# DUNE/larnd-sim

Measured on AMD Instinct MI355X. Metric: edep segments/s end-to-end (quench->ADC), module0 config, higher is better.
Workload: dtype f64

## Files before the change

### larnd-sim_amd/csrc/chain.hip

```cpp
#include <stdio.h>
#include <math.h>

#include <vector>

#include "ldsim_args.h"
#include <utility>

int seg_launch_max_pixels(ldsim_ctx*, int64_t, int64_t, int32_t*, unsigned long long*);
int seg_launch_get_pixels(ldsim_ctx*, int64_t, int64_t, int, int32_t*, int, int32_t*, int32_t*, int, double*, const int32_t*,
                          int32_t);
int sort_make_keys(ldsim_ctx*, const int32_t*, const int32_t*, int64_t, int32_t, int, int64_t, unsigned long long*,
                   int32_t*, unsigned long long*);
int sort_pairs(ldsim_ctx*, unsigned long long*, unsigned long long*, int32_t*, int32_t*, int64_t);
int sort_pairs_bits(ldsim_ctx*, unsigned long long*, unsigned long long*, int32_t*, int32_t*, int64_t, int, int);
int sort_compact_valid(ldsim_ctx*, const unsigned long long*, int64_t, unsigned long long*, int32_t*, unsigned int*);
int sort_exclusive_scan_i32(ldsim_ctx*, const int32_t*, int32_t*, int64_t);
int sort_heads(ldsim_ctx*, const unsigned long long*, int64_t, int32_t*);
int sort_fill_unique(ldsim_ctx*, const unsigned long long*, const int32_t*, const int32_t*, int64_t, int32_t, int32_t*,
                     int32_t*, int64_t*, int64_t);
int sort_batch_first(ldsim_ctx*, int64_t, int64_t, int32_t, int32_t*);
int sort_tmax_batch(ldsim_ctx*, int64_t, int64_t, int32_t, double*, int32_t*, unsigned long long*);
int gform_launch(ldsim_ctx* ctx, const CurArgs& a, unsigned long long* counters, int32_t** flags_out,
                 const int32_t** flag_list, const unsigned long long** flag_count);
int sort_compact_hits(ldsim_ctx*, const int32_t*, const int32_t*, const int32_t*, const int32_t*, const double*,
// ... 307 lines not shown
  a.pixels = nullptr;
  a.seg_begin = seg_begin;
  a.P = P;
  a.n_pairs = n_valid;
  a.out = d_waves;
  a.T = T;
  a.tmax_batch = d_tmax_b;
  a.batch0 = batch0;
  a.batch_first = d_first_b;
  a.counters = counters;
  a.only_flagged = nullptr;
  a.flag_stride = 0;
  CK(ldsim_ensure(ctx, SB_WIN, (size_t)n_valid * 8 + 8));
  a.win = (int32_t*)ctx->scratch[SB_WIN].p;
  HIPCHK(hipEventRecord(ctx->ev[1], st));
  bool split_timed = false, win_used = false;
  CK(run_tracks_current(ctx, a, n, counters, &split_timed, &win_used));
  HIPCHK(hipEventRecord(ctx->ev[2], st));

  CK(ldsim_ensure(ctx, SB_ADC, (size_t)U * A * 8));
  CK(ldsim_ensure(ctx, SB_TICKS, (size_t)U * A * 8));
  CK(ldsim_ensure(ctx, SB_DIGIT, (size_t)U * A * 8));
  CK(ldsim_ensure(ctx, SB_TPM, (size_t)U * M * 8));
  CK(ldsim_ensure(ctx, SB_PAIRPIX, (size_t)U * 8 + 16));
  if (want_fractions) CK(ldsim_ensure(ctx, SB_FRAC, (size_t)U * A * M * 8));
  int32_t* d_hitcnt = (int32_t*)ctx->scratch[SB_PAIRPIX].p;
  int32_t* d_hitoff = d_hitcnt + U;
  FeeArgs F{};
  F.c = ctx->d_consts;
  F.k = FEEK_FROM(h);
  F.U = U;
  F.upix = d_upix; F.ubatch = d_ubatch; F.uoff = d_uoff;
  F.pair_val = d_vals2; F.pair_key = d_keys2;
  F.P = P;
  F.track_starts = d_starts;
  F.waves = d_waves;
  F.win = win_used ? (const int32_t*)ctx->scratch[SB_WIN].p : nullptr;
  F.T = T;
  F.batch_first = d_first_b;
  F.batch0 = batch0;
  F.threshold = h.discrimination_threshold * 1.0;
  F.thr_table = tables_fit ? ctx->d_pix_thr : nullptr;
  F.gain_table = tables_fit ? ctx->d_pix_gain : nullptr;
  F.time_padding = 0.0;
  F.adc_list = (double*)ctx->scratch[SB_ADC].p;
  F.adc_ticks = (double*)ctx->scratch[SB_TICKS].p;
  F.adc_digit = (double*)ctx->scratch[SB_DIGIT].p;
  F.tpm = (int64_t*)ctx->scratch[SB_TPM].p;
  F.fractions = want_fractions ? (double*)ctx->scratch[SB_FRAC].p : nullptr;
  F.counters = counters;
  F.hit_count = d_hitcnt;
  F.debug = ctx->debug_phases;
  const bool noisy = h.reset_noise_charge != 0 || h.uncorrelated_noise_charge != 0 || h.discriminator_noise != 0;
  const bool keyed_inline = noisy && ctx->rng_keyed && !ctx->debug_rng_materialize;
  if (keyed_inline) {
    F.batch_keys = (const uint64_t*)ctx->d_batch_keys.p;
    F.rng_seed = ctx->rng_seed;
  } else if (noisy && ctx->rng_keyed) {
    const int nd = rng_fee_draws_per_pixel(h, h.n_time_ticks);
    CK(ldsim_ensure(ctx, SB_NOISE, (size_t)U * nd * 4));
    CK(ldsim_ensure(ctx, SB_NDRAWS, (size_t)U * 4 + 4));
    CK(rng_launch_fee_keyed_fill(ctx, d_ubatch, d_upix, U, nd, (float*)ctx->scratch[SB_NOISE].p));
    F.noise_z = (const float*)ctx->scratch[SB_NOISE].p;
    F.noise_nd = nd;
    F.n_draws = (int32_t*)ctx->scratch[SB_NDRAWS].p;
  } else if (noisy) {
// ... 46 lines not shown
```

### larnd-sim_amd/csrc/kernels_fee.hip

```cpp
#include <algorithm>
#include "ldsim_args.h"
#include "rng.h"

#define FEE_THREADS 256
#define FEE_SPAN 512
#define NT_MAX 4096
#define A_MAX 64
#define M_MAX 64


template <int CTRL, int ROW_MASK>
__device__ __forceinline__ double dpp_or_zero(double v) {
  const int lo = __builtin_amdgcn_update_dpp(0, __double2loint(v), CTRL, ROW_MASK, 0xF, true);
  const int hi = __builtin_amdgcn_update_dpp(0, __double2hiint(v), CTRL, ROW_MASK, 0xF, true);
  return __hiloint2double(hi, lo);
}
__device__ __forceinline__ double wave_incl_scan(double v, int lane) {
  v += dpp_or_zero<0x111, 0xF>(v);
  v += dpp_or_zero<0x112, 0xF>(v);
  v += dpp_or_zero<0x114, 0xF>(v);
  v += dpp_or_zero<0x118, 0xF>(v);
  v += dpp_or_zero<0x142, 0xA>(v);
  v += dpp_or_zero<0x143, 0xC>(v);
  return v;
// ... 120 lines not shown
      adc = q_sum + (double)za * s_unc;
      disc2 = (double)zb * s_disc;
      cur += 2;
    }
    if (adc < thr + disc2) {
      ic += reset_ticks;
      q_sum = z ? (double)zs.get(cur++) * s_reset : 0.0;
      true_q = 0;
      last_reset = ic;
      adc_busy = 0;
      continue;
    }
    if (lane == 0) {
      int crossing = ic < n_time_ticks - 1 ? ic : n_time_ticks - 1;
      int post = ic - crossing > 0 ? ic - crossing : 0;
      double tt = (crossing == NT) ? t_stop : crossing * tstep;
      hits[iadc].lr = last_reset;
      hits[iadc].b = integrate_end;
      hits[iadc].q = adc;
      hits[iadc].tq = true_q;
      hits[iadc].tick = tt + time_padding - 2 + post;
    }
    ic += reset_ticks;
    last_reset = ic;
    adc_busy = busy_ticks;
    q_sum = z ? (double)zs.get(cur++) * s_reset : 0.0;
    true_q = 0;
    iadc++;
  }
  *n_draws = cur;
  return iadc;
}

template <int THREADS, bool KEYED = false>
__device__ __forceinline__ void pixel_adc_body(const FeeArgs& F, const int64_t u, const int32_t* __restrict__ span ,
                                               const int s_cap) {
  const FeeK* c = &F.k;
  const int tid = threadIdx.x, lane = tid & 63, wv = tid >> 6;
  const int NT = c->n_time_ticks;
  const int A = c->max_adc_values, M = c->max_tracks_per_pixel;
  const double dt = c->time_sampling, rt = c->buffer_risetime;

  extern __shared__ double S[];
  __shared__ HitRec hits[A_MAX];
  __shared__ int s_start[M_MAX], s_w0[M_MAX], s_w1[M_MAX];
  __shared__ int64_t s_row[M_MAX];
  __shared__ double wtap[64], G[64];
  __shared__ int s_nh, s_trange[2];

  const int64_t p0 = F.uoff[u], p1 = F.uoff[u + 1];
  __shared__ int s_nvalid;
  if (tid == 0) s_nvalid = 0;
  __syncthreads();
  {
    int cnt = 0;
    for (int64_t p = p0 + tid; p < p1; p += THREADS) cnt += (F.pair_key[p] & 15ull) != 15ull;
    if (cnt) atomicAdd(&s_nvalid, cnt);
  }
  __syncthreads();
  const int n_valid = s_nvalid;
  const int n_slots = n_valid < M ? n_valid : M;
  const bool overflow = (p1 - p0) > n_slots;
  const int ubatch = F.ubatch[u];
  const int bfirst = F.batch_first[ubatch - F.batch0];
  if (tid < n_slots) {
    int32_t v = F.pair_val[p0 + tid];
    int r = v / F.P;
    s_start[tid] = (int)py_round(F.track_starts[r] / dt);
    s_row[tid] = p0 + tid;
    s_w0[tid] = F.win ? F.win[2 * (p0 + tid)] : 0;
    s_w1[tid] = F.win ? F.win[2 * (p0 + tid) + 1] : F.T;
    F.tpm[u * M + tid] = r - bfirst;
  } else if (tid < M) {
    F.tpm[u * M + tid] = -1;
  }
  const int ntap = rt > 0 ? (int)ceil(10 * rt / dt) : 0;
  if (tid <= ntap && rt > 0) {
    wtap[tid] = exp((-tid) * dt / rt) * (1 - exp(-dt / rt));
  }
  __syncthreads();
  if (tid == 0) {
    double acc = 0;
    for (int d = 0; d <= ntap; d++) {
      acc += (rt > 0 ? wtap[d] : 1.0) * dt;
      G[d] = acc;
    }
  }
  const int s_lo = span ? span[2 * u] : 0;
  const int s_hi = span ? min(s_lo + s_cap, NT) : NT;
  for (int t = tid; t < s_hi - s_lo; t += THREADS) S[t] = 0;
  if (tid == 0) {
    int t_lo = NT, t_hi = 0;
    for (int k = 0; k < n_slots; k++) {
      const int lo = max(s_start[k] + s_w0[k], 0), hi = min(s_start[k] + s_w1[k], NT);
      if (hi > lo) { t_lo = min(t_lo, lo); t_hi = max(t_hi, hi); }
    }
    s_trange[0] = t_lo;
    s_trange[1] = t_hi;
  }
  for (int k = 0; k < n_slots && !(F.debug & 0x10000); k++) {
    const int st = s_start[k];
    const int lo = max(st + s_w0[k], 0), hi = min(st + s_w1[k], NT);
    const float* wf = F.waves + s_row[k] * (int64_t)F.T - st;
    for (int t = lo + ((tid - lo) & (THREADS - 1)); t < hi; t += THREADS) S[t - s_lo] += (double)wf[t];
  }
  __syncthreads();
  if (wv == 0) {
    const double thr = F.thr_table ? F.thr_table[F.upix[u]] : F.threshold;
    int nd = 0;
    int nh = 0;
    if (F.debug & 0x20000) {
    } else if (KEYED) {
      const KeyedNoise zs{F.rng_seed, key_mix(F.batch_keys[ubatch], (uint64_t)(int64_t)F.upix[u])};
      nh = adc_scan(c, S, NT, 1 * c->time_interval1, thr, F.time_padding, lane, hits, wtap, ntap, zs, &nd, s_trange[0],
                    s_trange[1], s_lo, s_hi);
    } else {
      const TableNoise zs{F.noise_z ? F.noise_z + u * (int64_t)F.noise_nd : nullptr};
      nh = adc_scan(c, S, NT, 1 * c->time_interval1, thr, F.time_padding, lane, hits, wtap, ntap, zs, &nd, s_trange[0],
                    s_trange[1], s_lo, s_hi);
    }
    if (lane == 0) {
      s_nh = nh;
      if (F.n_draws) F.n_draws[u] = nd;
    }
  }
  __syncthreads();
  const int nh = s_nh;
  const double gain = F.gain_table ? F.gain_table[F.upix[u]] : c->gain * (1e-3 * (1e-6 * 1.0)) / 1.0;
  for (int h = tid; h < A; h += THREADS) {
    double q = h < nh ? hits[h].q : 0.0;
    F.adc_list[u * A + h] = q;
    F.adc_ticks[u * A + h] = h < nh ? hits[h].tick : 0.0;
    F.adc_digit[u * A + h] = digitize_one(c, q, gain);
  }
  if (tid == 0) {
    F.hit_count[u] = nh;
    if (overflow) stat_add(F.counters, 2, 1ull);
    if (nh) stat_add(F.counters, 3, (unsigned long long)nh);
  }
  if (F.fractions && !(F.debug & 0x40000)) {
    double* fr = F.fractions + u * (int64_t)A * M;
    for (int k = wv; k < n_slots; k += THREADS / 64) {
      const float* wf = F.waves + s_row[k] * (int64_t)F.T;
      const int st = s_start[k];
      for (int h = 0; h < nh; h++) {
        int lr = hits[h].lr, b = hits[h].b;
        int hi = b < NT - 1 ? b : NT - 1;
        const int j0 = max(lr, st + s_w0[k]), j1 = min(hi, st + s_w1[k] - 1);
        double acc = 0;
        for (int jc = j0 + ((lr + lane - j0) & 63); jc <= j1; jc += 64) {
          int it = jc - st;
          int d = b - jc;
          acc += (double)wf[it] * (rt > 0 ? G[d < ntap ? d : ntap] : dt);
        }
        acc = wave_sum(acc);
        if (lane == 0) fr[h * M + k] = hits[h].tq > 0 ? acc / hits[h].tq : acc;
      }
    }
  }
}

template <int THREADS, bool KEYED = false>
__global__ void __launch_bounds__(THREADS) pixel_adc_kernel(FeeArgs F) {
  if ((int64_t)blockIdx.x < F.U) pixel_adc_body<THREADS, KEYED>(F, (int64_t)blockIdx.x, nullptr, 0);
}
template <int THREADS, bool KEYED = false>
__global__ void __launch_bounds__(THREADS) pixel_adc_list_kernel(FeeArgs F, const int32_t* __restrict__ list,
                                                                const unsigned long long* __restrict__ count,
                                                                const int32_t* __restrict__ span, int s_cap) {
  const int64_t n = (int64_t)*count;
  for (int64_t i = blockIdx.x; i < n; i += gridDim.x) {
    pixel_adc_body<THREADS, KEYED>(F, (int64_t)list[i], span, s_cap);
    __syncthreads();
  }
}

__global__ void __launch_bounds__(256) fee_clear_fractions_kernel(int64_t U, const int32_t* __restrict__ hit_count,
                                                                 const int64_t* __restrict__ tpm, int A, int M, double* __restrict__ fr) {
  const int64_t u = blockIdx.x;
  if (u >= U) return;
  __shared__ int s_ns;
  if (threadIdx.x == 0) s_ns = 0;
  __syncthreads();
  if ((int)threadIdx.x < M && tpm[u * M + threadIdx.x] != -1) atomicAdd(&s_ns, 1);
  __syncthreads();
  const int nh = hit_count[u], ns = s_ns;
  double* row = fr + u * (int64_t)A * M;
  for (int h = 0; h < A; h++)
    for (int k = threadIdx.x; k < M; k += 256)
      if (!(h < nh && k < ns)) row[h * M + k] = 0.0;
}

extern "C++" int fee_clear_unwritten_fractions(ldsim_ctx* ctx, int64_t U, const int32_t* hit_count, const int64_t* tpm, double* fr) {
  if (U == 0) return 0;
  const LdsimConsts& h = ctx->h_consts;
  hipLaunchKernelGGL(fee_clear_fractions_kernel, dim3((unsigned)U), dim3(256), 0, ctx->stream, U, hit_count, tpm,
                     h.max_adc_values, h.max_tracks_per_pixel, fr);
  HIPCHK(hipGetLastError());
  return 0;
}

__global__ void __launch_bounds__(256) fee_span_kernel(FeeArgs F, int32_t* __restrict__ span, int32_t* __restrict__ lists ,
                                                       unsigned long long* __restrict__ counts ) {
  const FeeK* c = &F.k;
  const int64_t u = (int64_t)blockIdx.x * 256 + threadIdx.x;
  const int lane = threadIdx.x & 63;
  int cls = -1;
  if (u < F.U) {
    const int NT = c->n_time_ticks, M = c->max_tracks_per_pixel;
    const double dt = c->time_sampling;
    const int64_t p0 = F.uoff[u], p1 = F.uoff[u + 1];
    int n_slots = 0;
    for (int64_t p = p0; p < p1 && n_slots < M; p++) n_slots += (F.pair_key[p] & 15ull) != 15ull;
    int t_lo = NT, t_hi = 0;
    for (int k = 0; k < n_slots; k++) {
      const int r = F.pair_val[p0 + k] / F.P;
      const int st = (int)py_round(F.track_starts[r] / dt);
      const int w0 = F.win ? F.win[2 * (p0 + k)] : 0, w1 = F.win ? F.win[2 * (p0 + k) + 1] : F.T;
      const int lo = max(st + w0, 0), hi = min(st + w1, NT);
      if (hi > lo) { t_lo = min(t_lo, lo); t_hi = max(t_hi, hi); }
    }
    if (t_hi <= t_lo) { t_lo = 0; t_hi = 0; }
    span[2 * u] = t_lo;
    span[2 * u + 1] = t_hi;
    cls = (t_hi - t_lo <= FEE_SPAN) ? 0 : 1;
  }
  for (int cc = 0; cc < 2; cc++) {
    const unsigned long long m = __ballot(cls == cc);
    if (!m) continue;
    unsigned long long base = 0;
    if (lane == 0) base = atomicAdd(&counts[cc], (unsigned long long)__popcll(m));
    base = ((unsigned long long)(unsigned)__builtin_amdgcn_readfirstlane((int)(base >> 32)) << 32) |
           (unsigned)__builtin_amdgcn_readfirstlane((int)base);
    if (cls == cc) lists[(int64_t)cc * F.U + (int64_t)base + __popcll(m & ((1ull << lane) - 1ull))] = (int32_t)u;
  }
}

extern "C++" int fee_launch_chain(ldsim_ctx* ctx, const FeeArgs& F) {
  if (F.U == 0) return 0;
  const LdsimConsts& h = ctx->h_consts;
  if (h.n_time_ticks > NT_MAX || h.max_adc_values > A_MAX || h.max_tracks_per_pixel > M_MAX ||
      (h.buffer_risetime > 0 && 10 * h.buffer_risetime / h.time_sampling > 62)) {
    ldsim_set_error("FEE constants exceed the kernel's static tiles");
    return LDSIM_EINVAL;
  }
  const size_t full = (size_t)((h.n_time_ticks + 1) & ~1) * 8;
  if (F.batch_keys) {
    hipLaunchKernelGGL((pixel_adc_kernel<FEE_THREADS, true>), dim3((unsigned)F.U), dim3(FEE_THREADS), full, ctx->stream, F);
    HIPCHK(hipGetLastError());
    return 0;
  }
  const bool skip_idle = !F.noise_z && ((F.thr_table != nullptr) || F.threshold > 0);
  if (!skip_idle || !F.win || ctx->fee_one_class || h.n_time_ticks <= FEE_SPAN) {
    hipLaunchKernelGGL(pixel_adc_kernel<FEE_THREADS>, dim3((unsigned)F.U), dim3(FEE_THREADS), full, ctx->stream, F);
    HIPCHK(hipGetLastError());
    return 0;
  }
  int rc;
  if ((rc = ldsim_ensure(ctx, SB_SPAN, (size_t)F.U * 16 + 64))) return rc;
  int32_t* d_span = (int32_t*)ctx->scratch[SB_SPAN].p;
  int32_t* d_lists = d_span + 2 * F.U;
  unsigned long long* d_counts = (unsigned long long*)((char*)ctx->scratch[SB_SPAN].p + (((size_t)F.U * 16 + 15) & ~(size_t)15));
  HIPCHK(hipMemsetAsync(d_counts, 0, 16, ctx->stream));
  hipLaunchKernelGGL(fee_span_kernel, dim3((unsigned)((F.U + 255) / 256)), dim3(256), 0, ctx->stream, F, d_span, d_lists, d_counts);
  HIPCHK(hipGetLastError());
  const unsigned g_small = (unsigned)std::min<int64_t>(F.U, 256 * 24), g_big = (unsigned)std::min<int64_t>(F.U, 256 * 8);
  hipLaunchKernelGGL(pixel_adc_list_kernel<64>, dim3(g_small), dim3(64), (size_t)FEE_SPAN * 8, ctx->stream, F, d_lists,
                     d_counts, d_span, FEE_SPAN);
  HIPCHK(hipGetLastError());
  hipLaunchKernelGGL(pixel_adc_list_kernel<FEE_THREADS>, dim3(g_big), dim3(FEE_THREADS), full, ctx->stream, F,
                     d_lists + F.U, d_counts + 1, (const int32_t*)nullptr, 0);
  HIPCHK(hipGetLastError());
  return 0;
}

__global__ void track_pixel_map_kernel(int64_t* map, const int32_t* unique_pix, int64_t U, const int32_t* pixels,
                                       const int32_t* dist, int64_t S, int P, int max_distance, int M) {
  int64_t u = (int64_t)blockIdx.x * blockDim.x + threadIdx.x;
  if (u >= U) return;
  int32_t upix = unique_pix[u];
  int64_t* row = map + u * M;
  for (int target = 0; target < max_distance; target++)
    for (int64_t itrk = 0; itrk < S; itrk++)
      for (int ipix = 0; ipix < P; ipix++) {
        if (upix != pixels[itrk * P + ipix]) continue;
        if (dist[itrk * P + ipix] == target) {
          int imap = 0;
          while (imap < M) {
            if (row[imap] == itrk) { imap = -1; break; }
            if (row[imap] == -1) break;
            imap++;
          }
          if (imap >= 0 && imap < M) row[imap] = itrk;
        }
        break;
      }
}

__global__ void sum_pixel_signals_kernel(double* pixels_signals, const float* signals, const double* track_starts,
                                         const int64_t* pim, const int64_t* tpm, double* pts, double* overflow,
                                         int64_t S, int P, int T, int NT, int M, double dt) {
  int64_t pairi = blockIdx.x;
  int64_t itrk = pairi / P;
  int64_t pidx = pim[pairi];
// ... 127 lines not shown
```

### larnd-sim_amd/csrc/ldsim_abi.hip

```cpp
#include <stdarg.h>
#include <stdio.h>
#include <string.h>

#include <algorithm>
#include <cmath>
#include <new>
#include <vector>

#include "ldsim_args.h"

struct CurArgs;
struct FeeArgs;
int seg_launch_unpack(ldsim_ctx*, const LdsimTrackLayout*, int64_t);
int seg_launch_repack(ldsim_ctx*, const LdsimTrackLayout*, int64_t);
int seg_launch_quench_drift(ldsim_ctx*, int, int, int, int*);
int seg_launch_quench_drift_map(ldsim_ctx*, int, int*);
int seg_launch_max_pixels(ldsim_ctx*, int64_t, int64_t, int32_t*, unsigned long long*);
int seg_launch_get_pixels(ldsim_ctx*, int64_t, int64_t, int, int32_t*, int, int32_t*, int32_t*, int, double*, const int32_t*,
                          int32_t);
int seg_launch_time_intervals(ldsim_ctx*, int64_t, int64_t, double*, int32_t*);
int fee_launch_track_pixel_map(ldsim_ctx*, int64_t*, const int32_t*, int64_t, const int32_t*, const int32_t*, int64_t,
                               int, int, int);
int fee_launch_sum_pixel_signals(ldsim_ctx*, double*, const float*, const double*, const int64_t*, const int64_t*,
                                 double*, double*, int64_t, int, int, int, int);
// ... 168 lines not shown
    (void)ldsim_ctx_destroy(ctx);
    return rc;
  }
  *out = ctx;
  return 0;
}

extern "C" int ldsim_set_consts(ldsim_ctx* ctx, const LdsimConsts* consts) {
  LDSIM_ENTER(ctx);
  NEED(ctx && consts, "null argument");
  CK(light_join(ctx));
  NEED(consts->n_tpc >= 0 && consts->n_tpc <= LDSIM_MAX_TPC, "n_tpc out of range");
  if (memcmp(&ctx->h_consts, consts, sizeof(LdsimConsts)) != 0) ctx->wbuf_learned = 0;
  ctx->h_consts = *consts;
  HIPCHK(hipMemcpyAsync(ctx->d_consts, &ctx->h_consts, sizeof(LdsimConsts), hipMemcpyHostToDevice, ctx->stream));
  HIPCHK(hipStreamSynchronize(ctx->stream));
  return 0;
}

extern "C" int ldsim_ctx_destroy(ldsim_ctx* ctx) {
  if (!ctx) return 0;
  {
    const std::thread::id me = std::this_thread::get_id();
    std::thread::id none{};
    if (ctx->owner.load(std::memory_order_acquire) != me && !ctx->owner.compare_exchange_strong(none, me, std::memory_order_acq_rel)) {
      ldsim_set_error("ctx in use by another thread: not destroyed");
      return LDSIM_ESTATE;
    }
  }
  (void)hipSetDevice(ctx->device);
  if (ctx->stream) (void)hipStreamSynchronize(ctx->stream);
  void* ptrs[] = {ctx->d_consts, ctx->d_resp,      ctx->d_eff,    ctx->d_ch2tpc, ctx->d_lut_vis, ctx->d_lut_t0,
                  ctx->d_lut_t0avg, ctx->d_lut_td, ctx->seg_block.p, ctx->raw.p,  ctx->d_pix_thr, ctx->d_pix_gain,
                  ctx->d_glx, ctx->d_glw, ctx->light_flag_dev};
  for (void* p : ptrs)
    if (p) (void)hipFree(p);
  if (ctx->copy_stream) {
    (void)hipStreamSynchronize(ctx->copy_stream);
    (void)hipStreamDestroy(ctx->copy_stream);
  }
  if (ctx->light_stream) {
    (void)hipStreamSynchronize(ctx->light_stream);
    (void)hipStreamDestroy(ctx->light_stream);
  }
  if (ctx->tab_stream) {
    (void)hipStreamSynchronize(ctx->tab_stream);
    (void)hipStreamDestroy(ctx->tab_stream);
  }
  for (auto& e : ctx->tab_ev)
    if (e) (void)hipEventDestroy(e);
  if (ctx->ev_light_in) (void)hipEventDestroy(ctx->ev_light_in);
  if (ctx->ev_light_done) (void)hipEventDestroy(ctx->ev_light_done);
  for (auto& b : ctx->scratch)
    if (b.p) (void)hipFree(b.p);
  for (auto& b : ctx->out_alt)
    if (b.p) (void)hipFree(b.p);
  for (int i = 0; i < 8; i++)
    if (ctx->ev[i]) (void)hipEventDestroy(ctx->ev[i]);
  for (int i = 0; i < 4; i++)
    if (ctx->evl[i]) (void)hipEventDestroy(ctx->evl[i]);
  for (DevBuf* b : {&ctx->light_nph, &ctx->light_t0, &ctx->light_vox, &ctx->light_out, &ctx->light_tid, &ctx->light_tph,
                    &ctx->light_opc, &ctx->light_trk, &ctx->light_scint, &ctx->light_scint_tid, &ctx->light_scint_tph,
                    &ctx->light_disc, &ctx->light_resp, &ctx->light_resp_tid, &ctx->light_resp_tph, &ctx->light_w[0],
                    &ctx->light_w[1], &ctx->light_gain, &ctx->resp_pad, &ctx->light_tmax, &ctx->light_env, &ctx->light_xd, &ctx->light_wtid, &ctx->light_wtph, &ctx->light_wtid2})
    if (b->p) (void)hipFree(b->p);
  for (auto& b : ctx->light_tmp)
    if (b.p) (void)hipFree(b.p);
// ... 1385 lines not shown
```

### larnd-sim_amd/csrc/ldsim_args.h

```cpp
#pragma once
#include "ldsim_dev.h"

#define STAT_STRIPES 64
#define STAT_WORDS (16 * (1 + STAT_STRIPES))
#define STAT_BYTES (8 * STAT_WORDS)
#define MISC_BYTES (256 + STAT_BYTES + 256)
#ifdef __HIPCC__
__device__ __forceinline__ void stat_add(unsigned long long* counters, int i, unsigned long long v) {
  atomicAdd(&counters[16 * (1 + (blockIdx.x & (STAT_STRIPES - 1))) + i], v);
}
#endif
static inline void stat_sum(const unsigned long long* raw, unsigned long long* sum16) {
  for (int i = 0; i < 16; i++) {
    sum16[i] = raw[i];
    for (int s = 0; s < STAT_STRIPES; s++) sum16[i] += raw[16 * (1 + s) + i];
  }
}

struct CurArgs {
  SegStore s;
  const LdsimConsts* c;
  const double* resp;
  int32_t ni, nj, nk;
  int32_t k_first, k_last;
// ... 11 lines not shown
  double prune_log;
  double tail_log;
  int32_t debug_phases;
  int32_t numba_f32;
  int32_t split_max_items;
  unsigned long long* counters;
  int32_t* win;
  const int32_t* only_flagged;
  int32_t flag_stride;
  const int32_t* flag_list;
  const unsigned long long* flag_count;
};

struct FeeK {
  int32_t n_time_ticks, max_adc_values, max_tracks_per_pixel, pad;
  double time_sampling, buffer_risetime, clock_cycle, adc_hold_delay, reset_cycles, adc_busy_delay;
  double reset_noise_charge, uncorrelated_noise_charge, discriminator_noise;
  double v_pedestal, v_cm, v_ref, adc_counts, gain, time_interval1;
};
#define FEEK_FROM(h) FeeK{(h).n_time_ticks, (h).max_adc_values, (h).max_tracks_per_pixel, 0, (h).time_sampling, (h).buffer_risetime, \
                          (h).clock_cycle, (double)(h).adc_hold_delay, (double)(h).reset_cycles, (double)(h).adc_busy_delay,         \
                          (h).reset_noise_charge, (h).uncorrelated_noise_charge, (h).discriminator_noise, (h).v_pedestal, (h).v_cm, \
                          (h).v_ref, (double)(h).adc_counts, (h).gain, (h).time_interval[1]}

struct FeeArgs {
  const LdsimConsts* c;
  FeeK k;
  int64_t U;
  const int32_t* upix;
  const int32_t* ubatch;
  const int64_t* uoff;
  const int32_t* pair_val;
  const unsigned long long* pair_key;
  int32_t P;
  const double* track_starts;
  const float* waves;
  const int32_t* win;
  int32_t T;
  const int32_t* batch_first;
  int32_t batch0;
  double threshold;
  const double* thr_table;
  const double* gain_table;
  double time_padding;
  double* adc_list;
  double* adc_ticks;
  double* adc_digit;
  int64_t* tpm;
  double* fractions;
  unsigned long long* counters;
  int32_t* hit_count;
  const float* noise_z;
  int32_t noise_nd;
  int32_t* n_draws;
  const uint64_t* batch_keys;
  uint64_t rng_seed;
  int32_t debug;
};

int current_launch(ldsim_ctx* ctx, const CurArgs& args);
int current_mc_launch(ldsim_ctx* ctx, const CurArgs& args, int64_t n_seg);
int rng_ensure_states(ldsim_ctx* ctx, int64_t n);
int rng_fee_draws_per_pixel(const LdsimConsts& h, int NT);
int rng_launch_fee_noise(ldsim_ctx* ctx, int64_t U, int nd, float* z);
int rng_launch_advance(ldsim_ctx* ctx, int64_t U, const int32_t* n_draws);
int rng_launch_fee_keyed_fill(ldsim_ctx* ctx, const int32_t* ubatch, const int32_t* upix, int64_t U, int nd, float* z);
int fee_launch_chain(ldsim_ctx* ctx, const FeeArgs& F);
int split_launch_weights(ldsim_ctx* ctx, const CurArgs& args, void* items, void* hdr, void* corr, double* wbuf,
                         unsigned long long wbuf_cap, unsigned long long* cursor);
int split_launch_mac(ldsim_ctx* ctx, const CurArgs& args, void* items, void* hdr, void* corr, double* wbuf,
                     unsigned long long wbuf_cap, unsigned long long* cursor);
struct SplitArgs;
int qweights_launch(ldsim_ctx* ctx, const SplitArgs& S, int M, void* params);
int qpair_setup_launch(ldsim_ctx* ctx, const SplitArgs& S, int M, void* params, void* ginfo, void* maps);
size_t qpair_params_bytes(int64_t n_pairs);
int split_sizes(const ldsim_ctx* ctx, const CurArgs& args, size_t* item_bytes, size_t* hdr_bytes, size_t* corr_bytes);
```

### larnd-sim_amd/csrc/ldsim_dev.h

```cpp
#pragma once
#include <hip/hip_runtime.h>
#include <stdint.h>
#include <string.h>

#include <atomic>
#include <exception>
#include <thread>
#include <vector>

#include "../../include/ldsim.h"

#define LDSIM_WAVE 64

struct SegStore {
  double* f[LDSIM_NFIELDS - 1];
  int32_t* pixel_plane;
  int32_t* batch;
  int32_t store_code[LDSIM_NFIELDS];
  int64_t n;
  int64_t cap;
};

struct alignas(32) FieldMapNode {
  double e, dx, dy, dz;
// ... 88 lines not shown
  double* d_pix_thr = nullptr;
  double* d_pix_gain = nullptr;
  int64_t pix_table_n = 0;
  double* d_eff = nullptr;
  int32_t* d_ch2tpc = nullptr;
  int32_t n_light_ch = 0;
  DevBuf resp_pad;
  int32_t resp_pad_lo = 0, resp_pad_hi = -2;
  double quad_n0 = 3.4, quad_slope = 1.38;
  DevBuf light_wtid, light_wtph, light_wtid2;
  DevBuf light_xd;
  DevBuf light_env;
  int light_truth_lds = 1;
  DevBuf light_tmax;
  hipStream_t copy_stream = nullptr;
  DevBuf out_alt[7];
  int async_out = 0;
  int copy_pending = 0;
  int64_t out_gen = 0, pending_gen = 0;
  int light_eff_plain = 0;
  int light_incidence_scalar = 0;
  int mac_mode = 1;
  float *d_lut_vis = nullptr, *d_lut_t0 = nullptr, *d_lut_t0avg = nullptr, *d_lut_td = nullptr;
  int32_t lut_nx = 0, lut_ny = 0, lut_nz = 0, lut_ndet = 0, lut_nprof = 0;
  double prune_log = 23.0;
  double tail_log = 14.0;
  int trim_response = 1;
  double trim_response_log = 23.0;
  std::vector<double> h_resp_kmax;
  int debug_phases = 15;
  int debug_lds_b1_kb = 0;
  int debug_lds_pad_kb = 0;
  long long frac_clean_gen = -1;
  int fee_one_class = 0;
  int gform_chunks = 1;
  hipStream_t tab_stream = nullptr;
  hipEvent_t tab_ev[34] = {};
  int gform_wave_tables = 1;
  int debug_gform = 0;
  int split_kernels = 1;
  int wbuf_doubles_per_pair = 6144;
  int split_max_items = 0;
  int weights_mode = 2;
  int gform_max_support = 1000000000;
  int mc_current = 0;
  int numba_f32 = 0;
  double* d_glx = nullptr;
  double* d_glw = nullptr;
  int gl_nmax = 0;
  double wbuf_learned = 0;
  int64_t n_fallback = 0;
  SegStore seg{};
  DevBuf seg_block;
  DevBuf raw;
  LdsimTrackLayout seg_layout{};
  DevBuf scratch[40];
  std::vector<int32_t> h_batch;
  int seg_owner = 0;
  DevBuf light_nph, light_t0, light_vox;
  int32_t light_n_out = 0;
  int64_t light_n = -1;
  DevBuf light_out, light_tid, light_tph, light_opc, light_trk;
  int32_t light_sum_ndet = 0, light_sum_nticks = 0, light_sum_truth = 0;
  DevBuf light_tmp[9];
  int light_lazy_valid = 0, light_lazy_mt = 0, light_lazy_tick_bits = 16;
  long long light_lazy_nrec = 0, light_lazy_nticks = 0;
// ... 32 lines not shown
  FieldMapDesc h_fmap[LDSIM_MAX_TPC] = {};
  DevBuf fmap_nodes[LDSIM_MAX_TPC];
  FieldMapDesc* d_fmap = nullptr;
  int n_fmap = 0;
  int64_t fmap_gen = 0;
  int64_t drift_map_gen = -1;
  DevBuf fmap_view;
  int64_t fmap_view_cap = 0;
  void* comm = nullptr;
  int comm_rank = 0, comm_world = 0;
  DevBuf comm_tmp, hits_acc, hits_all;
  int64_t hits_acc_rows = 0;
  DevBuf cpt_acc[5], cpt_all[5], gv_send, gv_all;
  int64_t cpt_acc_n[5] = {0, 0, 0, 0, 0};
  int64_t cpt_acc_gen = -1;
  int64_t cpt_all_n[5] = {0, 0, 0, 0, 0};
  std::vector<int64_t> gv_all_n;
  int cpt_all_root = -1, cpt_all_src = -1;
  int gv_all_root = -1;
  LdsimChainStats stats{};
  LdsimChainStats stage_stats{};
  int64_t chain_U = 0, chain_hits = 0;
  int64_t cpt_n[4] = {0, 0, 0, 0};
  int64_t cpt_gen = -1;
  int want_fractions = 0;
  hipEvent_t ev[8] = {nullptr, nullptr, nullptr, nullptr, nullptr, nullptr, nullptr, nullptr};
  double ms_current = 0, ms_adc = 0, ms_total = 0;
  double ms_weights = 0, ms_mac = 0, ms_fallback = 0;
};

enum {
  SB_ACTIVE = 0, SB_NEIGH, SB_NRAD, SB_NLIST, SB_STARTS, SB_MISC, SB_KEYS, SB_KEYS2, SB_VALS, SB_VALS2,
  SB_SORTTMP, SB_PAIRSEG, SB_PAIRPIX, SB_HEADS, SB_UOFF, SB_UPIX, SB_UBATCH, SB_WAVES, SB_ADC, SB_TICKS,
  SB_DIGIT, SB_TPM, SB_FRAC, SB_HITS, SB_ITEMS, SB_HDR, SB_CORR, SB_WBUF, SB_NOISE, SB_NDRAWS, SB_PPAR, SB_CPT, SB_CPO, SB_WIN, SB_SPAN, SB_GMAPS
};

void ldsim_set_error(const char* fmt, ...);
static inline SegStore charge_store(const ldsim_ctx* ctx) {
  SegStore s = ctx->seg;
  if (ctx->drift_map_gen >= 0)
    for (int k = 0; k < LDSIM_NVIEW; k++) s.f[k] = (double*)ctx->fmap_view.p + (size_t)k * ctx->fmap_view_cap;
  return s;
}
int ldsim_ensure(ldsim_ctx* ctx, int slot, size_t bytes);
int ldsim_ensure_buf(ldsim_ctx* ctx, DevBuf* b, size_t bytes);
#define LDSIM_KEYED_STAGE_MSG \
  "%s draws random numbers, but the context is in keyed mode and this stage call carries no identity for its rows: " \
  "call ldsim_rng_seed for table mode"


struct CtxEnter {
  ldsim_ctx* c;
  bool ok;
  explicit CtxEnter(ldsim_ctx* ctx) : c(ctx), ok(true) {
    if (!c) return;
    const std::thread::id me = std::this_thread::get_id();
    if (c->owner.load(std::memory_order_acquire) == me) {
      c->owner_depth++;
      return;
    }
    std::thread::id none{};
    ok = c->owner.compare_exchange_strong(none, me, std::memory_order_acq_rel);
    if (ok) c->owner_depth = 1;
  }
  ~CtxEnter() {
    if (c && ok && --c->owner_depth == 0) c->owner.store(std::thread::id{}, std::memory_order_release);
  }
// ... 19 lines not shown
```

Baseline: 5.567 million.

## Precompute per-pixel FEE headers and slots in a setup kernel; cache tap tables

Adds a setup kernel that computes, for every unique pixel, its slot count, overflow flag, time range, batch info and per-track start and window records, and writes them to global header and slot arrays. The ADC kernels then read these precomputed records instead of doing an atomic valid-count pass, the track-start division and a serial time-range loop inside every block. The response tap and cumulative tables are computed once by a tiny kernel and cached across calls. The change also uses wavefront-only barriers for the 64-thread variant and prefetches the next header in the list kernel. In exchange it always launches an extra setup kernel and adds slot-array traffic.

Result: faster. 5.633 million (median of 6 runs) (+1.2%).

```diff
diff --git a/larnd-sim_amd/csrc/chain.hip b/larnd-sim_amd/csrc/chain.hip
--- a/larnd-sim_amd/csrc/chain.hip
+++ b/larnd-sim_amd/csrc/chain.hip
@@ -363,6 +363,7 @@
   F.U = U;
   F.upix = d_upix; F.ubatch = d_ubatch; F.uoff = d_uoff;
   F.pair_val = d_vals2; F.pair_key = d_keys2;
+  F.n_pairs = n_valid;
   F.P = P;
   F.track_starts = d_starts;
   F.waves = d_waves;
diff --git a/larnd-sim_amd/csrc/kernels_fee.hip b/larnd-sim_amd/csrc/kernels_fee.hip
--- a/larnd-sim_amd/csrc/kernels_fee.hip
+++ b/larnd-sim_amd/csrc/kernels_fee.hip
@@ -176,8 +176,60 @@
   return iadc;
 }
 
+#ifdef LDSIM_FEE_DEBUG
+#define FEEDBG(bit) ((F.debug & (bit)) != 0)
+#else
+#define FEEDBG(bit) false
+#endif
+
+__global__ void __launch_bounds__(64) fee_tables_kernel(double dt, double rt, double* __restrict__ tab) {
+  __shared__ double wtap[64];
+  const int tid = threadIdx.x;
+  const int ntap = rt > 0 ? (int)ceil(10 * rt / dt) : 0;
+  wtap[tid] = 0;
+  if (tid <= ntap && rt > 0) wtap[tid] = exp((-tid) * dt / rt) * (1 - exp(-dt / rt));
+  __syncthreads();
+  tab[tid] = wtap[tid];
+  tab[64 + tid] = 0;
+  __syncthreads();
+  if (tid == 0) {
+    double acc = 0;
+    for (int d = 0; d <= ntap; d++) {
+      acc += (rt > 0 ? wtap[d] : 1.0) * dt;
+      tab[64 + d] = acc;
+    }
+  }
+}
+
+struct __attribute__((aligned(32))) FeeHdr {
+  int32_t u;
+  int32_t n_slots;
+  int32_t overflow;
+  int32_t t_lo, t_hi;
+  int32_t s_lo;
+  int32_t bfirst;
+  int32_t ubatch;
+  int64_t p0;
+  int64_t pad;
+};
+struct __attribute__((aligned(16))) FeeSlot {
+  int32_t start;
+  int32_t w0, w1;
+  int32_t track;
+};
+
+template <int THREADS>
+__device__ __forceinline__ void fee_sync() {
+  if (THREADS == 64) {
+    __builtin_amdgcn_fence(__ATOMIC_ACQ_REL, "wavefront");
+    __builtin_amdgcn_wave_barrier();
+  } else {
+    __syncthreads();
+  }
+}
+
 template <int THREADS, bool KEYED = false>
-__device__ __forceinline__ void pixel_adc_body(const FeeArgs& F, const int64_t u, const int32_t* __restrict__ span ,
+__device__ __forceinline__ void pixel_adc_body(const FeeArgs& F, const FeeHdr& H, const FeeSlot* __restrict__ slots, const bool windowed,
                                                const int s_cap) {
   const FeeK* c = &F.k;
   const int tid = threadIdx.x, lane = tid & 63, wv = tid >> 6;
@@ -188,88 +240,55 @@
   extern __shared__ double S[];
   __shared__ HitRec hits[A_MAX];
   __shared__ int s_start[M_MAX], s_w0[M_MAX], s_w1[M_MAX];
-  __shared__ int64_t s_row[M_MAX];
   __shared__ double wtap[64], G[64];
-  __shared__ int s_nh, s_trange[2];
-
-  const int64_t p0 = F.uoff[u], p1 = F.uoff[u + 1];
-  __shared__ int s_nvalid;
-  if (tid == 0) s_nvalid = 0;
-  __syncthreads();
-  {
-    int cnt = 0;
-    for (int64_t p = p0 + tid; p < p1; p += THREADS) cnt += (F.pair_key[p] & 15ull) != 15ull;
-    if (cnt) atomicAdd(&s_nvalid, cnt);
-  }
-  __syncthreads();
-  const int n_valid = s_nvalid;
-  const int n_slots = n_valid < M ? n_valid : M;
-  const bool overflow = (p1 - p0) > n_slots;
-  const int ubatch = F.ubatch[u];
-  const int bfirst = F.batch_first[ubatch - F.batch0];
+  __shared__ int s_nh;
+
+  const int64_t u = H.u, p0 = H.p0;
+  const int n_slots = H.n_slots;
+  const int ntap = rt > 0 ? (int)ceil(10 * rt / dt) : 0;
   if (tid < n_slots) {
-    int32_t v = F.pair_val[p0 + tid];
-    int r = v / F.P;
-    s_start[tid] = (int)py_round(F.track_starts[r] / dt);
-    s_row[tid] = p0 + tid;
-    s_w0[tid] = F.win ? F.win[2 * (p0 + tid)] : 0;
-    s_w1[tid] = F.win ? F.win[2 * (p0 + tid) + 1] : F.T;
-    F.tpm[u * M + tid] = r - bfirst;
+    const FeeSlot sl = slots[p0 + tid];
+    s_start[tid] = sl.start;
+    s_w0[tid] = sl.w0;
+    s_w1[tid] = sl.w1;
+    F.tpm[u * M + tid] = sl.track;
   } else if (tid < M) {
     F.tpm[u * M + tid] = -1;
   }
-  const int ntap = rt > 0 ? (int)ceil(10 * rt / dt) : 0;
-  if (tid <= ntap && rt > 0) {
-    wtap[tid] = exp((-tid) * dt / rt) * (1 - exp(-dt / rt));
-  }
-  __syncthreads();
-  if (tid == 0) {
-    double acc = 0;
-    for (int d = 0; d <= ntap; d++) {
-      acc += (rt > 0 ? wtap[d] : 1.0) * dt;
-      G[d] = acc;
-    }
-  }
-  const int s_lo = span ? span[2 * u] : 0;
-  const int s_hi = span ? min(s_lo + s_cap, NT) : NT;
+  if (tid <= ntap) {
+    wtap[tid] = F.tab[tid];
+    G[tid] = F.tab[64 + tid];
+  }
+  const int s_lo = windowed ? H.s_lo : 0;
+  const int s_hi = windowed ? min(s_lo + s_cap, NT) : NT;
   for (int t = tid; t < s_hi - s_lo; t += THREADS) S[t] = 0;
-  if (tid == 0) {
-    int t_lo = NT, t_hi = 0;
-    for (int k = 0; k < n_slots; k++) {
-      const int lo = max(s_start[k] + s_w0[k], 0), hi = min(s_start[k] + s_w1[k], NT);
-      if (hi > lo) { t_lo = min(t_lo, lo); t_hi = max(t_hi, hi); }
-    }
-    s_trange[0] = t_lo;
-    s_trange[1] = t_hi;
-  }
-  for (int k = 0; k < n_slots && !(F.debug & 0x10000); k++) {
+  fee_sync<THREADS>();
+  for (int k = 0; k < n_slots && !FEEDBG(0x10000); k++) {
     const int st = s_start[k];
     const int lo = max(st + s_w0[k], 0), hi = min(st + s_w1[k], NT);
-    const float* wf = F.waves + s_row[k] * (int64_t)F.T - st;
+    const float* wf = F.waves + (p0 + k) * (int64_t)F.T - st;
     for (int t = lo + ((tid - lo) & (THREADS - 1)); t < hi; t += THREADS) S[t - s_lo] += (double)wf[t];
   }
-  __syncthreads();
+  fee_sync<THREADS>();
+  int nh = 0;
   if (wv == 0) {
     const double thr = F.thr_table ? F.thr_table[F.upix[u]] : F.threshold;
     int nd = 0;
-    int nh = 0;
-    if (F.debug & 0x20000) {
+    if (FEEDBG(0x20000)) {
     } else if (KEYED) {
-      const KeyedNoise zs{F.rng_seed, key_mix(F.batch_keys[ubatch], (uint64_t)(int64_t)F.upix[u])};
-      nh = adc_scan(c, S, NT, 1 * c->time_interval1, thr, F.time_padding, lane, hits, wtap, ntap, zs, &nd, s_trange[0],
-                    s_trange[1], s_lo, s_hi);
+      const KeyedNoise zs{F.rng_seed, key_mix(F.batch_keys[H.ubatch], (uint64_t)(int64_t)F.upix[u])};
+      nh = adc_scan(c, S, NT, 1 * c->time_interval1, thr, F.time_padding, lane, hits, wtap, ntap, zs, &nd, H.t_lo, H.t_hi, s_lo, s_hi);
     } else {
       const TableNoise zs{F.noise_z ? F.noise_z + u * (int64_t)F.noise_nd : nullptr};
-      nh = adc_scan(c, S, NT, 1 * c->time_interval1, thr, F.time_padding, lane, hits, wtap, ntap, zs, &nd, s_trange[0],
-                    s_trange[1], s_lo, s_hi);
+      nh = adc_scan(c, S, NT, 1 * c->time_interval1, thr, F.time_padding, lane, hits, wtap, ntap, zs, &nd, H.t_lo, H.t_hi, s_lo, s_hi);
     }
     if (lane == 0) {
-      s_nh = nh;
+      if (THREADS != 64) s_nh = nh;
       if (F.n_draws) F.n_draws[u] = nd;
     }
   }
-  __syncthreads();
-  const int nh = s_nh;
+  fee_sync<THREADS>();
+  if (THREADS != 64) nh = s_nh;
   const double gain = F.gain_table ? F.gain_table[F.upix[u]] : c->gain * (1e-3 * (1e-6 * 1.0)) / 1.0;
   for (int h = tid; h < A; h += THREADS) {
     double q = h < nh ? hits[h].q : 0.0;
@@ -279,13 +298,13 @@
   }
   if (tid == 0) {
     F.hit_count[u] = nh;
-    if (overflow) stat_add(F.counters, 2, 1ull);
+    if (H.overflow) stat_add(F.counters, 2, 1ull);
     if (nh) stat_add(F.counters, 3, (unsigned long long)nh);
   }
-  if (F.fractions && !(F.debug & 0x40000)) {
+  if (F.fractions && !FEEDBG(0x40000)) {
     double* fr = F.fractions + u * (int64_t)A * M;
     for (int k = wv; k < n_slots; k += THREADS / 64) {
-      const float* wf = F.waves + s_row[k] * (int64_t)F.T;
+      const float* wf = F.waves + (p0 + k) * (int64_t)F.T;
       const int st = s_start[k];
       for (int h = 0; h < nh; h++) {
         int lr = hits[h].lr, b = hits[h].b;
@@ -305,17 +324,25 @@
 }
 
 template <int THREADS, bool KEYED = false>
-__global__ void __launch_bounds__(THREADS) pixel_adc_kernel(FeeArgs F) {
-  if ((int64_t)blockIdx.x < F.U) pixel_adc_body<THREADS, KEYED>(F, (int64_t)blockIdx.x, nullptr, 0);
+__global__ void __launch_bounds__(THREADS) pixel_adc_kernel(FeeArgs F, const FeeHdr* __restrict__ hdr, const FeeSlot* __restrict__ slots) {
+  if ((int64_t)blockIdx.x < F.U) pixel_adc_body<THREADS, KEYED>(F, hdr[blockIdx.x], slots, false, 0);
 }
 template <int THREADS, bool KEYED = false>
-__global__ void __launch_bounds__(THREADS) pixel_adc_list_kernel(FeeArgs F, const int32_t* __restrict__ list,
+__global__ void __launch_bounds__(THREADS) pixel_adc_list_kernel(FeeArgs F, const FeeHdr* __restrict__ list,
                                                                 const unsigned long long* __restrict__ count,
-                                                                const int32_t* __restrict__ span, int s_cap) {
+                                                                const FeeSlot* __restrict__ slots, bool windowed, int s_cap) {
   const int64_t n = (int64_t)*count;
-  for (int64_t i = blockIdx.x; i < n; i += gridDim.x) {
-    pixel_adc_body<THREADS, KEYED>(F, (int64_t)list[i], span, s_cap);
-    __syncthreads();
+  int64_t i = blockIdx.x;
+  if (i >= n) return;
+  FeeHdr H = list[i];
+  while (true) {
+    const int64_t nx = i + gridDim.x;
+    const FeeHdr Hn = list[nx < n ? nx : i];
+    pixel_adc_body<THREADS, KEYED>(F, H, slots, windowed, s_cap);
+    if (nx >= n) break;
+    fee_sync<THREADS>();
+    H = Hn;
+    i = nx;
   }
 }
 
@@ -344,16 +371,19 @@
   return 0;
 }
 
-__global__ void __launch_bounds__(256) fee_span_kernel(FeeArgs F, int32_t* __restrict__ span, int32_t* __restrict__ lists ,
-                                                       unsigned long long* __restrict__ counts ) {
+__global__ void __launch_bounds__(256) fee_setup_kernel(FeeArgs F, FeeSlot* __restrict__ slots, FeeHdr* __restrict__ hdr ,
+                                                        unsigned long long* __restrict__ counts ) {
   const FeeK* c = &F.k;
   const int64_t u = (int64_t)blockIdx.x * 256 + threadIdx.x;
   const int lane = threadIdx.x & 63;
   int cls = -1;
+  FeeHdr H{};
   if (u < F.U) {
     const int NT = c->n_time_ticks, M = c->max_tracks_per_pixel;
     const double dt = c->time_sampling;
     const int64_t p0 = F.uoff[u], p1 = F.uoff[u + 1];
+    const int ubatch = F.ubatch[u];
+    const int bfirst = F.batch_first[ubatch - F.batch0];
     int n_slots = 0;
     for (int64_t p = p0; p < p1 && n_slots < M; p++) n_slots += (F.pair_key[p] & 15ull) != 15ull;
     int t_lo = NT, t_hi = 0;
@@ -363,12 +393,21 @@
       const int w0 = F.win ? F.win[2 * (p0 + k)] : 0, w1 = F.win ? F.win[2 * (p0 + k) + 1] : F.T;
       const int lo = max(st + w0, 0), hi = min(st + w1, NT);
       if (hi > lo) { t_lo = min(t_lo, lo); t_hi = max(t_hi, hi); }
-    }
-    if (t_hi <= t_lo) { t_lo = 0; t_hi = 0; }
-    span[2 * u] = t_lo;
-    span[2 * u + 1] = t_hi;
-    cls = (t_hi - t_lo <= FEE_SPAN) ? 0 : 1;
-  }
+      slots[p0 + k] = FeeSlot{st, w0, w1, r - bfirst};
+    }
+    H.u = (int32_t)u;
+    H.n_slots = n_slots;
+    H.overflow = (p1 - p0) > n_slots;
+    H.t_lo = t_lo;
+    H.t_hi = t_hi;
+    H.s_lo = t_hi <= t_lo ? 0 : t_lo;
+    H.bfirst = bfirst;
+    H.ubatch = ubatch;
+    H.p0 = p0;
+    if (!counts) hdr[u] = H;
+    else cls = (t_hi <= t_lo || t_hi - t_lo <= FEE_SPAN) ? 0 : 1;
+  }
+  if (!counts) return;
   for (int cc = 0; cc < 2; cc++) {
     const unsigned long long m = __ballot(cls == cc);
     if (!m) continue;
@@ -376,44 +415,54 @@
     if (lane == 0) base = atomicAdd(&counts[cc], (unsigned long long)__popcll(m));
     base = ((unsigned long long)(unsigned)__builtin_amdgcn_readfirstlane((int)(base >> 32)) << 32) |
            (unsigned)__builtin_amdgcn_readfirstlane((int)base);
-    if (cls == cc) lists[(int64_t)cc * F.U + (int64_t)base + __popcll(m & ((1ull << lane) - 1ull))] = (int32_t)u;
-  }
-}
-
-extern "C++" int fee_launch_chain(ldsim_ctx* ctx, const FeeArgs& F) {
-  if (F.U == 0) return 0;
+    if (cls == cc) hdr[(int64_t)cc * F.U + (int64_t)base + __popcll(m & ((1ull << lane) - 1ull))] = H;
+  }
+}
+
+extern "C++" int fee_launch_chain(ldsim_ctx* ctx, const FeeArgs& F0) {
+  if (F0.U == 0) return 0;
   const LdsimConsts& h = ctx->h_consts;
   if (h.n_time_ticks > NT_MAX || h.max_adc_values > A_MAX || h.max_tracks_per_pixel > M_MAX ||
       (h.buffer_risetime > 0 && 10 * h.buffer_risetime / h.time_sampling > 62)) {
     ldsim_set_error("FEE constants exceed the kernel's static tiles");
     return LDSIM_EINVAL;
   }
+  if (!ctx->d_fee_tab) HIPCHK(hipMalloc((void**)&ctx->d_fee_tab, 128 * sizeof(double)));
+  if (ctx->fee_tab_dt != h.time_sampling || ctx->fee_tab_rt != h.buffer_risetime) {
+    hipLaunchKernelGGL(fee_tables_kernel, dim3(1), dim3(64), 0, ctx->stream, h.time_sampling, h.buffer_risetime, ctx->d_fee_tab);
+    HIPCHK(hipGetLastError());
+    ctx->fee_tab_dt = h.time_sampling;
+    ctx->fee_tab_rt = h.buffer_risetime;
+  }
+  FeeArgs F = F0;
+  F.tab = ctx->d_fee_tab;
   const size_t full = (size_t)((h.n_time_ticks + 1) & ~1) * 8;
-  if (F.batch_keys) {
-    hipLaunchKernelGGL((pixel_adc_kernel<FEE_THREADS, true>), dim3((unsigned)F.U), dim3(FEE_THREADS), full, ctx->stream, F);
+  const bool skip_idle = !F.batch_keys && !F.noise_z && ((F.thr_table != nullptr) || F.threshold > 0);
+  const bool one_class = !skip_idle || !F.win || ctx->fee_one_class || h.n_time_ticks <= FEE_SPAN;
+  int rc;
+  const size_t hdr_bytes = (size_t)F.U * sizeof(FeeHdr) * (one_class ? 1 : 2);
+  if ((rc = ldsim_ensure(ctx, SB_SPAN, hdr_bytes + 64))) return rc;
+  if ((rc = ldsim_ensure(ctx, SB_FEESLOT, (size_t)F.n_pairs * sizeof(FeeSlot) + 16))) return rc;
+  FeeHdr* d_hdr = (FeeHdr*)ctx->scratch[SB_SPAN].p;
+  FeeSlot* d_slots = (FeeSlot*)ctx->scratch[SB_FEESLOT].p;
+  unsigned long long* d_counts = one_class ? nullptr : (unsigned long long*)((char*)ctx->scratch[SB_SPAN].p + hdr_bytes);
+  if (d_counts) HIPCHK(hipMemsetAsync(d_counts, 0, 16, ctx->stream));
+  hipLaunchKernelGGL(fee_setup_kernel, dim3((unsigned)((F.U + 255) / 256)), dim3(256), 0, ctx->stream, F, d_slots, d_hdr, d_counts);
+  HIPCHK(hipGetLastError());
+  if (one_class) {
+    if (F.batch_keys)
+      hipLaunchKernelGGL((pixel_adc_kernel<FEE_THREADS, true>), dim3((unsigned)F.U), dim3(FEE_THREADS), full, ctx->stream, F, d_hdr, d_slots);
+    else
+      hipLaunchKernelGGL(pixel_adc_kernel<FEE_THREADS>, dim3((unsigned)F.U), dim3(FEE_THREADS), full, ctx->stream, F, d_hdr, d_slots);
     HIPCHK(hipGetLastError());
     return 0;
   }
-  const bool skip_idle = !F.noise_z && ((F.thr_table != nullptr) || F.threshold > 0);
-  if (!skip_idle || !F.win || ctx->fee_one_class || h.n_time_ticks <= FEE_SPAN) {
-    hipLaunchKernelGGL(pixel_adc_kernel<FEE_THREADS>, dim3((unsigned)F.U), dim3(FEE_THREADS), full, ctx->stream, F);
-    HIPCHK(hipGetLastError());
-    return 0;
-  }
-  int rc;
-  if ((rc = ldsim_ensure(ctx, SB_SPAN, (size_t)F.U * 16 + 64))) return rc;
-  int32_t* d_span = (int32_t*)ctx->scratch[SB_SPAN].p;
-  int32_t* d_lists = d_span + 2 * F.U;
-  unsigned long long* d_counts = (unsigned long long*)((char*)ctx->scratch[SB_SPAN].p + (((size_t)F.U * 16 + 15) & ~(size_t)15));
-  HIPCHK(hipMemsetAsync(d_counts, 0, 16, ctx->stream));
-  hipLaunchKernelGGL(fee_span_kernel, dim3((unsigned)((F.U + 255) / 256)), dim3(256), 0, ctx->stream, F, d_span, d_lists, d_counts);
-  HIPCHK(hipGetLastError());
   const unsigned g_small = (unsigned)std::min<int64_t>(F.U, 256 * 24), g_big = (unsigned)std::min<int64_t>(F.U, 256 * 8);
-  hipLaunchKernelGGL(pixel_adc_list_kernel<64>, dim3(g_small), dim3(64), (size_t)FEE_SPAN * 8, ctx->stream, F, d_lists,
-                     d_counts, d_span, FEE_SPAN);
+  hipLaunchKernelGGL(pixel_adc_list_kernel<64>, dim3(g_small), dim3(64), (size_t)FEE_SPAN * 8, ctx->stream, F, d_hdr,
+                     d_counts, d_slots, true, FEE_SPAN);
   HIPCHK(hipGetLastError());
   hipLaunchKernelGGL(pixel_adc_list_kernel<FEE_THREADS>, dim3(g_big), dim3(FEE_THREADS), full, ctx->stream, F,
-                     d_lists + F.U, d_counts + 1, (const int32_t*)nullptr, 0);
+                     d_hdr + F.U, d_counts + 1, d_slots, false, 0);
   HIPCHK(hipGetLastError());
   return 0;
 }
diff --git a/larnd-sim_amd/csrc/ldsim_abi.hip b/larnd-sim_amd/csrc/ldsim_abi.hip
--- a/larnd-sim_amd/csrc/ldsim_abi.hip
+++ b/larnd-sim_amd/csrc/ldsim_abi.hip
@@ -224,7 +224,7 @@
   if (ctx->stream) (void)hipStreamSynchronize(ctx->stream);
   void* ptrs[] = {ctx->d_consts, ctx->d_resp,      ctx->d_eff,    ctx->d_ch2tpc, ctx->d_lut_vis, ctx->d_lut_t0,
                   ctx->d_lut_t0avg, ctx->d_lut_td, ctx->seg_block.p, ctx->raw.p,  ctx->d_pix_thr, ctx->d_pix_gain,
-                  ctx->d_glx, ctx->d_glw, ctx->light_flag_dev};
+                  ctx->d_glx, ctx->d_glw, ctx->light_flag_dev, ctx->d_fee_tab};
   for (void* p : ptrs)
     if (p) (void)hipFree(p);
   if (ctx->copy_stream) {
diff --git a/larnd-sim_amd/csrc/ldsim_args.h b/larnd-sim_amd/csrc/ldsim_args.h
--- a/larnd-sim_amd/csrc/ldsim_args.h
+++ b/larnd-sim_amd/csrc/ldsim_args.h
@@ -67,6 +67,7 @@
   const int64_t* uoff;
   const int32_t* pair_val;
   const unsigned long long* pair_key;
+  int64_t n_pairs;
   int32_t P;
   const double* track_starts;
   const float* waves;
@@ -91,6 +92,7 @@
   const uint64_t* batch_keys;
   uint64_t rng_seed;
   int32_t debug;
+  const double* tab;
 };
 
 int current_launch(ldsim_ctx* ctx, const CurArgs& args);
diff --git a/larnd-sim_amd/csrc/ldsim_dev.h b/larnd-sim_amd/csrc/ldsim_dev.h
--- a/larnd-sim_amd/csrc/ldsim_dev.h
+++ b/larnd-sim_amd/csrc/ldsim_dev.h
@@ -144,6 +144,8 @@
   int debug_lds_b1_kb = 0;
   int debug_lds_pad_kb = 0;
   long long frac_clean_gen = -1;
+  double* d_fee_tab = nullptr;
+  double fee_tab_dt = 0, fee_tab_rt = -1;
   int fee_one_class = 0;
   int gform_chunks = 1;
   hipStream_t tab_stream = nullptr;
@@ -242,7 +244,7 @@
 enum {
   SB_ACTIVE = 0, SB_NEIGH, SB_NRAD, SB_NLIST, SB_STARTS, SB_MISC, SB_KEYS, SB_KEYS2, SB_VALS, SB_VALS2,
   SB_SORTTMP, SB_PAIRSEG, SB_PAIRPIX, SB_HEADS, SB_UOFF, SB_UPIX, SB_UBATCH, SB_WAVES, SB_ADC, SB_TICKS,
-  SB_DIGIT, SB_TPM, SB_FRAC, SB_HITS, SB_ITEMS, SB_HDR, SB_CORR, SB_WBUF, SB_NOISE, SB_NDRAWS, SB_PPAR, SB_CPT, SB_CPO, SB_WIN, SB_SPAN, SB_GMAPS
+  SB_DIGIT, SB_TPM, SB_FRAC, SB_HITS, SB_ITEMS, SB_HDR, SB_CORR, SB_WBUF, SB_NOISE, SB_NDRAWS, SB_PPAR, SB_CPT, SB_CPO, SB_WIN, SB_SPAN, SB_GMAPS, SB_FEESLOT
 };
 
 void ldsim_set_error(const char* fmt, ...);
```
